# Icelk/fractal-renderer

Measured on AMD Instinct MI355X. Metric: pixel_iterations_per_sec, higher is better.
Workload: dtype f64

## Files before the change

### fractal-renderer_amd/_native.py

```python
import ctypes as C
import os

PKG_DIR = os.path.dirname(os.path.abspath(__file__))
LIB_PATH = os.path.join(PKG_DIR, "libfractal_hip.so")

FR_OK, FR_ERR_INVALID_ARGUMENT, FR_ERR_BUFFER_TOO_SMALL, FR_ERR_NO_DEVICE, FR_ERR_HIP = 0, 1, 2, 3, 4
STATUS_NAMES = {
    1: "FR_ERR_INVALID_ARGUMENT",
    2: "FR_ERR_BUFFER_TOO_SMALL",
    3: "FR_ERR_NO_DEVICE",
    4: "FR_ERR_HIP",
    5: "FR_ERR_UNSUPPORTED_ALGO",
}


class FractalHipError(RuntimeError):
    def __init__(self, code, message):
        super().__init__("%s: %s" % (STATUS_NAMES.get(code, "fr_status %d" % code), message))
        self.code = code


class Imaginary(C.Structure):

    _fields_ = [("re", C.c_double), ("im", C.c_double)]
# ... 241 lines not shown
    "fr_wide_to_double": (C.c_int, [C.c_void_p, C.c_uint32, C.POINTER(C.c_double), C.POINTER(C.c_double)]),
    "fr_wide_from_decimal": (C.c_int, [C.c_char_p, C.c_void_p, C.c_uint32]),
    "fr_render_rows_pt_wide": (
        C.c_int, [C.POINTER(fr_config), _WIDE, C.c_uint32, C.c_uint32, C.c_int, C.c_void_p, C.c_size_t]),
    "fr_render_rows_pt_wide_device": (
        C.c_int, [C.POINTER(fr_config), _WIDE, C.c_uint32, C.c_uint32, C.c_int, C.c_void_p, C.c_size_t, C.c_void_p]),
    "fr_escape_rows_pt_wide": (C.c_int, [C.POINTER(fr_config), _WIDE, C.c_uint32, C.c_uint32, C.c_void_p, C.c_void_p]),
    "fr_escape_rows_pt_wide_state_device": (
        C.c_int,
        [C.POINTER(fr_config), _WIDE, C.c_uint32, C.c_uint32, C.c_void_p, C.c_void_p, C.c_void_p, C.c_void_p, C.c_void_p],
    ),
    "fr_escape_extend_pt_wide_device": (
        C.c_int,
        [C.POINTER(fr_config), _WIDE, C.c_uint32, C.c_uint32, C.c_uint32, C.c_void_p, C.c_void_p, C.c_void_p, C.c_void_p,
         C.c_void_p],
    ),
    "fr_escape_rows_pt_wide_state": (
        C.c_int, [C.POINTER(fr_config), _WIDE, C.c_uint32, C.c_uint32, C.c_void_p, C.c_void_p, C.c_void_p, C.c_void_p]),
    "fr_escape_extend_pt_wide": (
        C.c_int,
        [C.POINTER(fr_config), _WIDE, C.c_uint32, C.c_uint32, C.c_uint32, C.c_void_p, C.c_void_p, C.c_void_p, C.c_void_p],
    ),
    "fr_debug_reference_orbit_wide": (
        C.c_int, [C.POINTER(fr_config), _WIDE, C.c_int, C.c_void_p, C.c_size_t, C.POINTER(C.c_uint32)]),
    "fr_render_rows_pt_bla": (
        C.c_int,
        [C.POINTER(fr_config), C.POINTER(Imaginary), _WIDE, C.c_int, C.c_uint32, C.c_uint32, C.c_int, C.c_void_p, C.c_size_t]),
    "fr_render_rows_pt_bla_device": (
        C.c_int,
        [C.POINTER(fr_config), C.POINTER(Imaginary), _WIDE, C.c_int, C.c_uint32, C.c_uint32, C.c_int, C.c_void_p, C.c_size_t,
         C.c_void_p],
    ),
    "fr_escape_rows_pt_bla": (
        C.c_int, [C.POINTER(fr_config), C.POINTER(Imaginary), _WIDE, C.c_int, C.c_uint32, C.c_uint32, C.c_void_p, C.c_void_p]),
    "fr_escape_rows_pt_bla_device": (
        C.c_int,
        [C.POINTER(fr_config), C.POINTER(Imaginary), _WIDE, C.c_int, C.c_uint32, C.c_uint32, C.c_void_p, C.c_void_p, C.c_void_p],
    ),
    "fr_debug_bla_table": (
        C.c_int,
        [C.POINTER(fr_config), C.POINTER(Imaginary), _WIDE, C.c_int, C.c_int, C.c_uint32, C.c_void_p, C.c_size_t,
         C.POINTER(C.c_uint32)],
    ),
    "fr_debug_bla_count": (
        C.c_int,
        [C.POINTER(fr_config), C.POINTER(Imaginary), _WIDE, C.c_int, C.c_uint32, C.c_uint32, C.POINTER(C.c_uint64),
         C.POINTER(C.c_uint64)],
    ),
    "fr_debug_bla_cache": (C.c_int, [C.POINTER(C.c_uint32)]),
    "fr_render_rows_pt_scaled": (
        C.c_int, [C.POINTER(fr_config), _WIDE, C.c_int, C.c_uint32, C.c_uint32, C.c_int, C.c_void_p, C.c_size_t]),
    "fr_render_rows_pt_scaled_device": (
        C.c_int, [C.POINTER(fr_config), _WIDE, C.c_int, C.c_uint32, C.c_uint32, C.c_int, C.c_void_p, C.c_size_t, C.c_void_p]),
    "fr_escape_rows_pt_scaled": (C.c_int, [C.POINTER(fr_config), _WIDE, C.c_int, C.c_uint32, C.c_uint32, C.c_void_p, C.c_void_p]),
    "fr_escape_rows_pt_scaled_device": (
        C.c_int, [C.POINTER(fr_config), _WIDE, C.c_int, C.c_uint32, C.c_uint32, C.c_void_p, C.c_void_p, C.c_void_p]),
    "fr_debug_bla_table_scaled": (
        C.c_int, [C.POINTER(fr_config), _WIDE, C.c_int, C.c_int, C.c_uint32, C.c_void_p, C.c_size_t, C.POINTER(C.c_uint32)]),
    "fr_debug_pt_scaled_count": (
        C.c_int, [C.POINTER(fr_config), _WIDE, C.c_int, C.c_uint32, C.c_uint32, C.POINTER(C.c_uint64), C.POINTER(C.c_uint64)]),
    "fr_colour_rows_device": (
        C.c_int,
        [C.POINTER(fr_config), C.c_void_p, C.c_int, C.c_void_p, C.c_size_t, C.c_int, C.c_void_p, C.c_size_t, C.c_void_p],
    ),
    "fr_count_iterations": (
        C.c_int,
        [C.POINTER(fr_config), C.c_int, C.c_uint32, C.c_uint32, C.c_uint32, C.c_uint32, C.POINTER(C.c_uint64),
         C.POINTER(C.c_uint64)],
    ),
    "fr_set_profiling": (C.c_int, [C.c_int]),
    "fr_last_kernel_ms": (C.c_int, [C.POINTER(C.c_float)]),
    "fr_set_tile": (C.c_int, [C.c_int]),
    "fr_set_loop_mode": (C.c_int, [C.c_int]),
    "fr_debug_loop_plan": (C.c_int, [C.POINTER(fr_config), C.c_int, C.POINTER(C.c_uint32), C.POINTER(C.c_double),
                                     C.POINTER(C.c_uint32)]),
    "fr_debug_set_spec_maxlen": (C.c_int, [C.c_uint32]),
    "fr_debug_spec_maxlen": (C.c_int, [C.POINTER(fr_config), C.c_int, C.POINTER(C.c_uint32)]),
    "fr_set_palette": (C.c_int, [C.c_int]),
    "fr_set_cycle_shortcut": (C.c_int, [C.c_int]),
    "fr_set_refill_policy": (C.c_int, [C.c_int, C.c_int]),
    "fr_debug_math": (C.c_int, [C.c_int, C.c_void_p, C.c_void_p, C.c_size_t]),
    "fr_debug_set_queue_trace": (C.c_int, [C.c_void_p]),
    "fr_debug_set_two_pass_capacity": (C.c_int, [C.c_uint32]),
}

_lib = None


def load():
    global _lib
    if _lib is not None:
        return _lib
    if not os.path.exists(LIB_PATH):
        raise ImportError(
            "%s is missing — build it first (python -c 'import __graft_entry__ as g; g.build()'); "
            "this package has no CPU fallback" % LIB_PATH
        )
    lib = C.CDLL(LIB_PATH)
    for name, (restype, argtypes) in PROTOTYPES.items():
        fn = getattr(lib, name)
        fn.restype = restype
        fn.argtypes = argtypes
    _lib = lib
    return lib


def check(rc):
    if rc != FR_OK:
        msg = load().fr_last_error()
        raise FractalHipError(rc, msg.decode() if msg else "")
```

### fractal-renderer_amd/build.py

```python
import hashlib
import os
import shutil
import subprocess

PKG_DIR = os.path.dirname(os.path.abspath(__file__))
CSRC = os.path.join(PKG_DIR, "csrc")
LIB_PATH = os.path.join(PKG_DIR, "libfractal_hip.so")
ID_PATH = LIB_PATH + ".id"
KERNEL_SOURCES = ["fr_kernels.hip", "fr_bla.hip", "fr_scaled.hip"]
SOURCES = KERNEL_SOURCES + ["fr_dispatch.hip", "fr_api.hip", "fr_host.hip", "fr_multi.hip", "fr_fern.hip",
                            "fr_dd.hip", "fr_pt.hip", "fr_wide.hip", "fr_ss.hip"]
DEPS = SOURCES + ["fr_kernels.h", "fr_launch.h", "fr_ctx.h", "fr_wide.h", "fr_bla.h", "fr_math.h", "fr_colour.h", "fr_log2_table.inc",
                  os.path.join("..", "..", "include", "fractal_hip.h")]
HIPCC_FLAGS = [
    "--offload-arch=gfx950",
    "-O3",
    "-std=c++17",
    "-ffp-contract=off",
    "-fno-fast-math",
    "-fPIC",
    "-shared",
    "-Wall",
    "-Wextra",
    "-pthread",
]
LINK_FLAGS = ["-ldl"]


def find_hipcc():
    for cand in (os.environ.get("HIPCC"), "/opt/rocm/bin/hipcc", shutil.which("hipcc")):
        if cand and os.path.exists(cand):
            return cand
    raise RuntimeError("hipcc not found (set HIPCC or install ROCm under /opt/rocm)")


def source_id():
    h = hashlib.sha256()
    h.update(" ".join(HIPCC_FLAGS + LINK_FLAGS).encode())
    for d in DEPS:
        h.update(d.encode())
        with open(os.path.join(CSRC, d), "rb") as f:
            h.update(f.read())
    return h.hexdigest()[:16]


def built_id():
    try:
        with open(ID_PATH) as f:
            return f.read().strip()
    except OSError:
        return None


def is_stale():
    return not os.path.exists(LIB_PATH) or built_id() != source_id()


def build_extension(force=False, verbose=False):
    if not force and not is_stale():
        return LIB_PATH
    sid = source_id()
    cmd = ([find_hipcc()] + HIPCC_FLAGS + ['-DFR_BUILD_ID="%s"' % sid, "-o", LIB_PATH]
           + [os.path.join(CSRC, s) for s in SOURCES] + LINK_FLAGS)
    if verbose:
        print(" ".join(cmd))
    if os.path.exists(ID_PATH):
        os.remove(ID_PATH)
    subprocess.run(cmd, check=True, cwd=CSRC)
    with open(ID_PATH, "w") as f:
        f.write(sid + "\n")
    return LIB_PATH


if __name__ == "__main__":
    print(build_extension(force=True, verbose=True))
```

### fractal-renderer_amd/csrc/fr_ctx.h

```cpp
#ifndef FR_CTX_H
#define FR_CTX_H

#include <hip/hip_runtime.h>

#include <atomic>
#include <cstddef>
#include <cstdint>
#include <memory>
#include <condition_variable>
#include <mutex>
#include <string>
#include <thread>
#include <vector>

#include "../../include/fractal_hip.h"
#include "fr_kernels.h"
#include "fr_wide.h"

namespace fr {

int fail(int code, const char *what);
int fail(int code, const std::string &what);
int fail_hip(hipError_t e, const char *what);
const std::string &last_error();
// ... 92 lines not shown
    struct CopyPool *copy_pool = nullptr;
    int reserve_stage(size_t bytes);

    std::mutex pt_mu;
    std::shared_ptr<PtOrbit> pt_orbit;
    std::shared_ptr<BlaTable> bla_table;

    int create(int device);
    void destroy();
    int reserve(Scratch &s, size_t bytes);
    int event(size_t k, hipEvent_t *out);
    int acquire_palette(PaletteSlot **out);
    void release_palette(PaletteSlot *slot, hipStream_t stream);
    int acquire_surv(size_t bytes, SurvSlot **out);
    void release_surv(SurvSlot *slot, hipStream_t stream);
};

void fill_params(const fr_config *cfg, const Opts &o, fr_kparams &p);
void plan_loop(const fr_config *cfg, int precision, const Opts &o, fr_kparams &p);
void rows_params(const fr_config *cfg, const Opts &o, uint32_t y0, uint32_t y1, unsigned channels, fr_kparams &p);

int render_device(Ctx &ctx, const fr_config *cfg, fr_kparams &p, int precision, const Opts &o, void *d_out,
                  hipStream_t stream);

int render_block_cyclic(Ctx &ctx, const fr_config *cfg, int precision, const Opts &o, uint32_t block_rows,
                        uint32_t first_block, uint32_t block_stride, uint32_t max_blocks, int dest_is_image,
                        void *d_out, size_t out_len, hipStream_t stream, uint64_t *rows_written);

int check_precision(int precision);
int check_rows(const fr_config *cfg, uint32_t y0, uint32_t y1);
int check_channels(int channels);

int check_dd(const fr_config *cfg, const fr_imaginary *pos_lo);
int check_pt(const fr_config *cfg, const fr_imaginary *pos_lo);
int check_precision_or_deep(const fr_config *cfg, int precision);
int check_precision_lo(const fr_config *cfg, int precision, const fr_imaginary *pos_lo);

struct Centre {
    const fr_imaginary *pos_lo;
    const fr_wide_centre *wide;
    bool scaled = false;
    double lo_re() const { return pos_lo ? pos_lo->re : 0.0; }
    double lo_im() const { return pos_lo ? pos_lo->im : 0.0; }
    int check(const fr_config *cfg, int precision) const;
};

int prof_begin(hipStream_t stream);
int prof_end(hipStream_t stream, const char *kernel_name);

int render_deep_device(Ctx &ctx, int precision, const fr_config *cfg, const Centre &c, const Opts &o, uint32_t y0, uint32_t y1,
                       unsigned bpp, void *d_out, hipStream_t stream);
int render_rows_device(const fr_config *cfg, int precision, const Centre &c, uint32_t y0, uint32_t y1, void *d_out, size_t out_len,
                       void *hip_stream, unsigned bytes_per_pixel, const fr_render_opts *opts);
int escape_rows(const fr_config *cfg, int precision, const Centre &c, uint32_t y0, uint32_t y1, double *z, uint32_t *iters,
                unsigned zw);
int launch_pt(Ctx &ctx, const fr_config *cfg, const Centre &c, const fr_kparams &p, int mode, const fr_kout &out,
              hipStream_t stream, const char **kernel_name);

struct PtOrbitView {
    const double2 *x = nullptr, *k = nullptr;
    uint32_t x_last = 0, k_last = 0;
};
int pt_orbit_view(Ctx &ctx, const fr_config *cfg, const Centre &c, std::shared_ptr<PtOrbit> &keep, PtOrbitView &v);
void pt_host_orbit(const fr_config *cfg, const Centre &c, int which, std::vector<double> &out);

void decide_kernel(Ctx &ctx, const fr_config *cfg, int precision, uint32_t y0, uint32_t y1, Opts &o, hipStream_t stream,
                   bool allow_async);

int primary(Ctx **out);
Ctx *primary_if_created();

struct LifeShared {
    LifeShared();
    ~LifeShared();
};
struct LifeExclusive {
    LifeExclusive();
    ~LifeExclusive();
};


class ChunkPinner {
  public:
    ChunkPinner(uint8_t *out, size_t need, bool portable, const std::vector<size_t> *byte_order = nullptr);
    ~ChunkPinner();
    size_t chunks() const { return bounds_.size() - 1; }
    size_t bound(size_t k) const { return bounds_[k]; }
    size_t chunk_of(size_t byte) const;
    bool pin(size_t k);
    bool next(size_t &a, size_t &b, bool &pinned);
    void release();
    static size_t chunk_end(const uint8_t *out, size_t need, size_t a);
    double t_touch = 0.0, t_reg = 0.0;

  private:
    uint8_t *out_;
    size_t need_, pos_ = 0;
    unsigned flags_;
    std::vector<size_t> bounds_;
    std::unique_ptr<std::atomic<int>[]> state_;
    std::vector<char> pinned_;
    std::thread toucher_;
    std::mutex reg_mu_;
    std::vector<uint8_t *> regs_;
};
void prefault(void *ptr, size_t len);
void destroy_copy_pool(CopyPool *pool);

struct Profiling {
    bool enabled = false;
    bool have = false;
    hipEvent_t e0 = nullptr, e1 = nullptr;
    const char *kernel = "";
    ~Profiling();
};
Profiling &profiling();


template <class Launch>
int host_rgb(uint8_t *out, size_t need, Launch &&launch) {
    LifeShared ls;
    Ctx *ctx;
    int rc = primary(&ctx);
    if (rc != FR_OK) return rc;
    std::lock_guard<std::mutex> lk(ctx->mu);
    rc = ctx->reserve(ctx->rgb, need);
    if (rc == FR_OK) rc = launch(*ctx, ctx->rgb.ptr, ctx->stream);
    if (rc != FR_OK) return rc;
    HIP_TRY(hipMemcpyAsync(out, ctx->rgb.ptr, need, hipMemcpyDeviceToHost, ctx->stream));
    HIP_TRY(hipStreamSynchronize(ctx->stream));
    return FR_OK;
}

template <class Launch>
int host_raw(double *z, size_t zb, uint32_t *iters, size_t ib, double *dz, uint32_t *m, bool upload, Launch &&launch) {
    LifeShared ls;
    Ctx *ctx;
    int rc = primary(&ctx);
    if (rc != FR_OK) return rc;
    std::lock_guard<std::mutex> lk(ctx->mu);
    if (z) rc = ctx->reserve(ctx->z, dz ? 2 * zb : zb);
    if (rc == FR_OK && iters) rc = ctx->reserve(ctx->iters, m ? 2 * ib : ib);
    if (rc != FR_OK) return rc;
    char *const d_z = z ? static_cast<char *>(ctx->z.ptr) : nullptr, *const d_iters = iters ? static_cast<char *>(ctx->iters.ptr) : nullptr;
    const struct {
        void *host, *dev;
        size_t bytes;
    } arrays[4] = {{z, d_z, zb}, {iters, d_iters, ib}, {dz, dz ? d_z + zb : nullptr, zb}, {m, m ? d_iters + ib : nullptr, ib}};
    if (upload)
        for (const auto &a : arrays)
            if (a.host) HIP_TRY(hipMemcpyAsync(a.dev, a.host, a.bytes, hipMemcpyHostToDevice, ctx->stream));
    rc = launch(*ctx, static_cast<double *>(arrays[0].dev), static_cast<uint32_t *>(arrays[1].dev), static_cast<double *>(arrays[2].dev),
                static_cast<uint32_t *>(arrays[3].dev), ctx->stream);
    if (rc != FR_OK) return rc;
    for (const auto &a : arrays)
        if (a.host) HIP_TRY(hipMemcpyAsync(a.host, a.dev, a.bytes, hipMemcpyDeviceToHost, ctx->stream));
    HIP_TRY(hipStreamSynchronize(ctx->stream));
    return FR_OK;
}

void multi_shutdown_locked();

}

int fr_host_render_rows(const fr_config *cfg, int precision, uint32_t y0, uint32_t y1, uint8_t *out, size_t out_len,
                        unsigned bytes_per_pixel, const fr_render_opts *opts);
int fr_host_render_rows_deep(const fr_config *cfg, int precision, const fr::Centre &c, uint32_t y0, uint32_t y1, uint8_t *out,
                             size_t out_len, unsigned bytes_per_pixel, const fr_render_opts *opts);

#endif
```

### fractal-renderer_amd/csrc/fr_host.hip

```cpp
#include <sys/mman.h>
#include <unistd.h>

#include <immintrin.h>

#include <atomic>
#include <chrono>
#include <condition_variable>
#include <cstdio>
#include <cstdlib>
#include <cstring>
#include <thread>
#include <vector>

#include "fr_ctx.h"

#ifndef MADV_HUGEPAGE
#define MADV_HUGEPAGE 14
#endif

namespace fr {

namespace {

constexpr size_t kPage = 4096;
constexpr size_t kHuge = (size_t)2 << 20;
constexpr size_t kChunk = (size_t)64 << 20;
constexpr size_t kPinThreshold = (size_t)16 << 20;
constexpr size_t kStageMax = (size_t)40 << 20;
constexpr size_t kSdmaMin = (size_t)5 << 20;

double now_ms() {
    using namespace std::chrono;
    return duration<double, std::milli>(steady_clock::now().time_since_epoch()).count();
}

bool trace_enabled() {
    static const bool on = getenv("FR_TRACE") != nullptr;
    return on;
}

int touch_threads() {
    static const int n = [] {
        const char *e = getenv("FR_TOUCH_THREADS");
        if (e && atoi(e) > 0) return atoi(e) > 64 ? 64 : atoi(e);
        long cpus = sysconf(_SC_NPROCESSORS_ONLN);
        return (int)(cpus >= 16 ? 8 : cpus >= 4 ? cpus / 2 : 1);
    }();
    return n;
}

bool looks_resident(uint8_t *p, size_t len) {
    uint8_t *a = reinterpret_cast<uint8_t *>(reinterpret_cast<uintptr_t>(p) & ~(kPage - 1));
    const size_t span = (size_t)(p + len - a);
    const size_t pages = (span + kPage - 1) / kPage;
    std::vector<unsigned char> vec(pages);
    if (mincore(a, span, vec.data()) != 0) return true;
    size_t missing = 0;
    for (size_t k = 0; k < pages; k++) missing += !(vec[k] & 1);
    return missing * 16 < pages;
}

void touch_range(uint8_t *p, size_t len) {
    volatile uint8_t *v = p;
    for (size_t k = 0; k < len; k += kPage) v[k] = v[k];
    if (len) v[len - 1] = v[len - 1];
}

}

void prefault(void *ptr, size_t len) {
    uint8_t *p = static_cast<uint8_t *>(ptr);
    uint8_t *ha = reinterpret_cast<uint8_t *>((reinterpret_cast<uintptr_t>(p) + kHuge - 1) & ~(kHuge - 1));
    uint8_t *hb = reinterpret_cast<uint8_t *>(reinterpret_cast<uintptr_t>(p + len) & ~(kHuge - 1));
    if (hb > ha) (void)madvise(ha, (size_t)(hb - ha), MADV_HUGEPAGE);
    const int T = touch_threads();
    if (T <= 1 || len < 8 * kHuge) {
        touch_range(p, len);
        return;
    }
    std::atomic<size_t> next{0};
    const size_t piece = 4 * kHuge;
    auto work = [&] {
        for (;;) {
            const size_t a = next.fetch_add(piece);
            if (a >= len) break;
            touch_range(p + a, a + piece < len ? piece : len - a);
        }
    };
    std::vector<std::thread> th;
    for (int t = 1; t < T; t++) th.emplace_back(work);
    work();
    for (auto &t : th) t.join();
}


size_t ChunkPinner::chunk_end(const uint8_t *out, size_t need, size_t a) {
    const size_t left = need - a;
    size_t b = a + (left <= kChunk + kChunk / 4 ? kChunk / 4 : kChunk);
    if (b >= need) return need;
    b -= (reinterpret_cast<uintptr_t>(out) + b) & (kPage - 1);
    return b > a ? b : need;
}

ChunkPinner::ChunkPinner(uint8_t *out, size_t need, bool portable, const std::vector<size_t> *byte_order)
    : out_(out), need_(need), flags_(portable ? hipHostRegisterPortable : hipHostRegisterDefault) {
    for (size_t a = 0; a < need;) {
        const size_t b = chunk_end(out, need, a);
        bounds_.push_back(a);
        a = b;
    }
    bounds_.push_back(need);
    const size_t n = chunks();
    state_.reset(new std::atomic<int>[n]);
    const bool fresh = !looks_resident(out, need < 4 * kChunk ? need : 4 * kChunk);
    for (size_t k = 0; k < n; k++) state_[k].store(fresh ? 0 : 1);
    pinned_.assign(n, 0);
    if (fresh) {
        std::vector<size_t> order;
        std::vector<char> seen(n, 0);
        if (byte_order)
            for (size_t byte : *byte_order) {
                const size_t k = chunk_of(byte < need ? byte : need - 1);
                if (!seen[k]) seen[k] = 1, order.push_back(k);
            }
        for (size_t k = 0; k < n; k++)
            if (!seen[k]) order.push_back(k);
        toucher_ = std::thread([this, order] {
            for (size_t k : order) {
                prefault(out_ + bounds_[k], bounds_[k + 1] - bounds_[k]);
                state_[k].store(1, std::memory_order_release);
            }
        });
    }
}

size_t ChunkPinner::chunk_of(size_t byte) const {
    size_t lo = 0, hi = chunks();
    while (hi - lo > 1) {
        const size_t mid = (lo + hi) / 2;
        if (bounds_[mid] <= byte) lo = mid;
        else hi = mid;
    }
    return lo;
}

bool ChunkPinner::pin(size_t k) {
    if (pinned_[k]) return pinned_[k] == 1;
    const uintptr_t base = reinterpret_cast<uintptr_t>(out_);
    const size_t a = bounds_[k], b = bounds_[k + 1];
    const double t0 = now_ms();
    while (state_[k].load(std::memory_order_acquire) == 0) std::this_thread::yield();
    const double t1 = now_ms();
    uint8_t *ra = reinterpret_cast<uint8_t *>((base + a) & ~(kPage - 1));
    uint8_t *rb = b < need_ ? out_ + b : reinterpret_cast<uint8_t *>((base + b + kPage - 1) & ~(kPage - 1));
    const hipError_t re = hipHostRegister(ra, (size_t)(rb - ra), flags_);
    bool ok = re == hipSuccess;
    if (!ok) {
        (void)hipGetLastError();
        ok = re == hipErrorHostMemoryAlreadyRegistered;
    }
    const double t2 = now_ms();
    {
        std::lock_guard<std::mutex> lk(reg_mu_);
        if (re == hipSuccess) regs_.push_back(ra);
        t_touch += t1 - t0;
        t_reg += t2 - t1;
    }
    pinned_[k] = ok ? 1 : 2;
    return ok;
}

bool ChunkPinner::next(size_t &a, size_t &b, bool &pinned) {
    if (pos_ >= chunks()) return false;
    a = bounds_[pos_];
    b = bounds_[pos_ + 1];
    pinned = pin(pos_);
    pos_++;
    return true;
}

void ChunkPinner::release() {
    if (toucher_.joinable()) toucher_.join();
    for (uint8_t *r : regs_) (void)hipHostUnregister(r);
    regs_.clear();
}

ChunkPinner::~ChunkPinner() { release(); }


struct CopyPool {
    struct Piece {
        uint8_t *dst;
        const uint8_t *src;
        size_t len;
        int kind;
    };
    std::vector<std::thread> threads;
    std::mutex m;
    std::condition_variable work_cv, done_cv;
    std::vector<Piece> pieces;
    size_t outstanding = 0;
    bool stop = false;

    explicit CopyPool(int helpers) {
        for (int t = 0; t < helpers; t++) threads.emplace_back([this] { loop(); });
    }
    static void run(const Piece &p) {
        if (p.kind == 0) memcpy(p.dst, p.src, p.len);
        else prefault(p.dst, p.len);
    }
    void loop() {
        for (;;) {
            Piece p;
            {
                std::unique_lock<std::mutex> lk(m);
                work_cv.wait(lk, [&] { return stop || !pieces.empty(); });
                if (pieces.empty()) return;
                p = pieces.back();
                pieces.pop_back();
            }
            run(p);
            std::lock_guard<std::mutex> lk(m);
            if (--outstanding == 0) done_cv.notify_all();
        }
    }
    void post(const std::vector<Piece> &ps) {
        if (ps.empty()) return;
        {
            std::lock_guard<std::mutex> lk(m);
            for (const Piece &p : ps) pieces.push_back(p);
            outstanding += ps.size();
        }
        work_cv.notify_all();
    }
    void wait() {
        for (;;) {
            Piece p;
            {
                std::lock_guard<std::mutex> lk(m);
                if (pieces.empty()) break;
                p = pieces.back();
                pieces.pop_back();
            }
            run(p);
            std::lock_guard<std::mutex> lk(m);
            --outstanding;
        }
        std::unique_lock<std::mutex> lk(m);
        done_cv.wait(lk, [&] { return outstanding == 0; });
    }
    ~CopyPool() {
        {
            std::lock_guard<std::mutex> lk(m);
            stop = true;
        }
        work_cv.notify_all();
        for (auto &t : threads) t.join();
    }
};

void destroy_copy_pool(CopyPool *pool) { delete pool; }

namespace {

// ... 114 lines not shown
    CopyPool *pool = helpers > 0 ? ctx.copy_pool : nullptr;

    auto spread = [&](uint8_t *dst, const uint8_t *src, size_t len, int kind) {
        if (!pool || len < ((size_t)1 << 20)) {
            CopyPool::run(CopyPool::Piece{dst, src, len, kind});
            return;
        }
        const size_t parts = (size_t)helpers + 1;
        const size_t piece = ((len + parts - 1) / parts + 4095) & ~(size_t)4095;
        std::vector<CopyPool::Piece> ps;
        for (size_t off = piece; off < len; off += piece)
            ps.push_back(CopyPool::Piece{dst + off, src ? src + off : nullptr, off + piece < len ? piece : len - off, kind});
        pool->post(ps);
        CopyPool::run(CopyPool::Piece{dst, src, piece < len ? piece : len, kind});
        pool->wait();
    };
    if (rc == FR_OK && err == hipSuccess && need >= ((size_t)1 << 20) && !looks_resident(out, need)) spread(out, nullptr, need, 1);
    const double t_touched = now_ms();
    for (uint32_t b = 0; b < nb && rc == FR_OK && err == hipSuccess; b++) {
        const uint32_t ya = y0 + b * band_rows, yb = ya + band_rows < y1 ? ya + band_rows : y1;
        const size_t a = row_bytes * (size_t)(ya - y0), len = row_bytes * (size_t)(yb - ya);
        if (len < kSdmaMin) {
            err = wait_flag(ctx.stage_flags + b, seq0 + b, (b & 1) ? ctx.stream2 : ctx.stream);
        } else {
            hipEvent_t ec;
            rc = ctx.event(b, &ec);
            if (rc != FR_OK) break;
            err = wait_event(ec);
        }
        if (err != hipSuccess) {
            what = "waiting for a band to arrive in the staging buffer";
            break;
        }
        spread(out + a, stage + a, len, 0);
    }
    if (rc != FR_OK || err != hipSuccess) {
        (void)hipStreamSynchronize(ctx.stream);
        (void)hipStreamSynchronize(ctx.stream2);
        (void)hipStreamSynchronize(ctx.copy_stream);
    }
    if (trace) {
        fprintf(stderr, "[fr_host] staged %zu bytes in %u bands: enqueued at %.3f ms, first touch until %.3f, copied out at %.3f", need, nb,
                t_enqueued - t_start, t_touched - t_start, now_ms() - t_start);
        if (t_enqueued - t_start > 1.0) {
            fprintf(stderr, "  [marks:");
            for (double m : marks) fprintf(stderr, " %.3f", m);
            fprintf(stderr, "]");
        }
        fprintf(stderr, "\n");
    }
    if (rc != FR_OK) return rc;
    if (err != hipSuccess) return fail_hip(err, what);
    return FR_OK;
}


int host_render_rows(Ctx &ctx, const fr_config *cfg, int precision, const Opts &o, uint32_t y0, uint32_t y1,
                     uint8_t *out, unsigned bpp) {
    const size_t row_bytes = (size_t)bpp * cfg->width;
    const size_t need = row_bytes * (size_t)(y1 - y0);
    if (need <= kStageMax && staging_enabled() && ctx.reserve_stage(need > ((size_t)40 << 20) ? need : (size_t)40 << 20) == FR_OK)
        return host_render_staged(ctx, cfg, precision, o, y0, y1, out, bpp);
    int rc = ctx.reserve(ctx.rgb, need);
    if (rc != FR_OK) return rc;
    uint8_t *scratch = static_cast<uint8_t *>(ctx.rgb.ptr);
    const bool trace = trace_enabled();
    const double t_start = now_ms();

    const Opts *use_opts = &o;
    auto render_on = [&](hipStream_t st, uint32_t ya, uint32_t yb, uint8_t *dst) -> int {
        fr_kparams p;
        rows_params(cfg, *use_opts, ya, yb, bpp, p);
        return render_device(ctx, cfg, p, precision, *use_opts, dst, st);
    };

    if (need < kPinThreshold) {
        rc = render_on(ctx.stream, y0, y1, scratch);
        if (rc != FR_OK) return rc;
        HIP_TRY(hipMemcpyAsync(out, scratch, need, hipMemcpyDeviceToHost, ctx.stream));
        HIP_TRY(hipStreamSynchronize(ctx.stream));
        return FR_OK;
    }

    Opts ob = o;
    decide_kernel(ctx, cfg, precision, y0, y1, ob, ctx.stream, true);
    const int pending_sample = ob.pending_sample;
    ob.pending_sample = -1;
    use_opts = &ob;
    struct Band {
        uint32_t ya, yb;
        size_t a, b;
    };
    std::vector<Band> bands;
    {
        uint32_t ya = y0;
        size_t a = 0;
        while (ya < y1) {
            const size_t target = ChunkPinner::chunk_end(out, need, a);
            uint64_t rows = (target - a + row_bytes - 1) / row_bytes;
            rows = (rows + 7) / 8 * 8;
            const uint32_t yb = (uint32_t)((uint64_t)ya + rows < y1 ? ya + rows : y1);
            const size_t b = row_bytes * (size_t)(yb - y0);
            bands.push_back(Band{ya, yb, a, b});
            ya = yb;
            a = b;
        }
    }
    std::vector<size_t> order;
    {
        size_t pow2 = 1;
        int bits = 0;
        while (pow2 < bands.size()) pow2 <<= 1, bits++;
        for (size_t i = 0; i < pow2; i++) {
            size_t r = 0;
            for (int k = 0; k < bits; k++) r |= ((i >> k) & 1u) << (bits - 1 - k);
            if (r < bands.size()) order.push_back(r);
        }
    }
    hipError_t err = hipSuccess;
    const char *what = "";
    std::vector<hipEvent_t> tk, tc;
    hipEvent_t t_zero = nullptr;
    if (trace && hipEventCreate(&t_zero) == hipSuccess) (void)hipEventRecord(t_zero, ctx.stream);
    for (size_t i = 0; i < order.size() && rc == FR_OK && err == hipSuccess; i++) {
        const Band &bd = bands[order[i]];
        hipStream_t st = (i & 1) ? ctx.stream2 : ctx.stream;
        rc = render_on(st, bd.ya, bd.yb, scratch + bd.a);
        if (rc != FR_OK) break;
        hipEvent_t e;
        rc = ctx.event(i, &e);
        if (rc != FR_OK) break;
        if ((err = hipEventRecord(e, st)) != hipSuccess) what = "hipEventRecord";
        if (t_zero) {
            hipEvent_t te;
            if (hipEventCreate(&te) == hipSuccess) {
                (void)hipEventRecord(te, st);
                tk.push_back(te);
            }
        }
    }
    ctx.post_sample(pending_sample, (order.size() & 1) ? ctx.stream : ctx.stream2);
    const double t_launched = now_ms();

    std::vector<size_t> byte_order;
    for (size_t k : order) byte_order.push_back(bands[k].a);
    ChunkPinner pinner(out, need, false, &byte_order);
    for (size_t i = 0; i < order.size() && rc == FR_OK && err == hipSuccess; i++) {
        const Band &bd = bands[order[i]];
        hipEvent_t e;
        rc = ctx.event(i, &e);
        if (rc != FR_OK) break;
        bool waited = false;
        for (size_t pos = bd.a; pos < bd.b && err == hipSuccess;) {
            const size_t k = pinner.chunk_of(pos);
            const size_t end = pinner.bound(k + 1) < bd.b ? pinner.bound(k + 1) : bd.b;
            if (pinner.pin(k)) {
                if (!waited) {
                    if ((err = hipStreamWaitEvent(ctx.copy_stream, e, 0)) != hipSuccess) what = "hipStreamWaitEvent";
                    waited = true;
                }
                if (err == hipSuccess &&
                    (err = hipMemcpyAsync(out + pos, scratch + pos, end - pos, hipMemcpyDeviceToHost, ctx.copy_stream)) != hipSuccess)
                    what = "hipMemcpyAsync";
            } else {
                if ((err = hipEventSynchronize(e)) != hipSuccess) what = "hipEventSynchronize";
                else if ((err = hipMemcpy(out + pos, scratch + pos, end - pos, hipMemcpyDeviceToHost)) != hipSuccess) what = "hipMemcpy";
            }
            pos = end;
        }
        if (t_zero) {
            hipEvent_t te;
            if (hipEventCreate(&te) == hipSuccess) {
                (void)hipEventRecord(te, ctx.copy_stream);
                tc.push_back(te);
            }
        }
    }
    const double t_enqueued = now_ms();
    hipError_t e1 = hipStreamSynchronize(ctx.stream);
    const hipError_t e1b = hipStreamSynchronize(ctx.stream2);
    if (e1 == hipSuccess) e1 = e1b;
    hipError_t e2 = hipStreamSynchronize(ctx.copy_stream);
    const double t_synced = now_ms();
    pinner.release();
    if (trace)
        fprintf(stderr,
                "[fr_host] %zu bytes: kernels enqueued at %.2f ms, waited for first touch %.2f, pinning %.2f, copies "
                "enqueued at %.2f, drained at %.2f, unpinned at %.2f\n",
                need, t_launched - t_start, pinner.t_touch, pinner.t_reg, t_enqueued - t_start, t_synced - t_start,
                now_ms() - t_start);
    if (t_zero) {
        fprintf(stderr, "[fr_host]   band kernels done at (ms):");
        for (hipEvent_t e : tk) {
            float ms = 0.0f;
            (void)hipEventElapsedTime(&ms, t_zero, e);
            fprintf(stderr, " %.1f", ms);
            (void)hipEventDestroy(e);
        }
        fprintf(stderr, "\n[fr_host]   chunk copies done at (ms):");
        for (hipEvent_t e : tc) {
            float ms = 0.0f;
            (void)hipEventElapsedTime(&ms, t_zero, e);
            fprintf(stderr, " %.1f", ms);
            (void)hipEventDestroy(e);
        }
        fprintf(stderr, "\n");
        (void)hipEventDestroy(t_zero);
    }
    if (rc != FR_OK) return rc;
    if (err != hipSuccess) return fail_hip(err, what);
    if (e1 != hipSuccess) return fail_hip(e1, "hipStreamSynchronize(stream)");
    if (e2 != hipSuccess) return fail_hip(e2, "hipStreamSynchronize(copy_stream)");
    return FR_OK;
}

}

using namespace fr;

int fr_host_render_rows(const fr_config *cfg, int precision, uint32_t y0, uint32_t y1, uint8_t *out, size_t out_len,
                        unsigned bpp, const fr_render_opts *opts) {
    int rc = check_rows(cfg, y0, y1);
    if (rc != FR_OK) return rc;
    if (precision == FR_PRECISION_DD || precision == FR_PRECISION_PT)
        return fr_host_render_rows_deep(cfg, precision, Centre{}, y0, y1, out, out_len, bpp, opts);
    rc = check_precision(precision);
    Opts o;
    if (rc == FR_OK) rc = resolve_opts(opts, o);
    if (rc != FR_OK) return rc;
    const size_t need = (size_t)bpp * cfg->width * (size_t)(y1 - y0);
    if (need == 0) return FR_OK;
    if (!out) return fail(FR_ERR_INVALID_ARGUMENT, "out is NULL");
    if (out_len < need)
        return fail(FR_ERR_BUFFER_TOO_SMALL, bpp == 4 ? "out_len < 4*width*(y1-y0)" : "out_len < 3*width*(y1-y0)");
    LifeShared ls;
    Ctx *ctx;
    rc = primary(&ctx);
    if (rc != FR_OK) return rc;
    std::lock_guard<std::mutex> lk(ctx->mu);
    return host_render_rows(*ctx, cfg, precision, o, y0, y1, out, bpp);
}

int fr_host_render_rows_deep(const fr_config *cfg, int precision, const Centre &c, uint32_t y0, uint32_t y1, uint8_t *out,
                             size_t out_len, unsigned bpp, const fr_render_opts *opts) {
    int rc = check_rows(cfg, y0, y1);
    if (rc == FR_OK) rc = c.check(cfg, precision);
    Opts o;
    if (rc == FR_OK) rc = resolve_opts(opts, o);
    if (rc != FR_OK) return rc;
    const size_t need = (size_t)bpp * cfg->width * (size_t)(y1 - y0);
    if (need == 0) return FR_OK;
    if (!out) return fail(FR_ERR_INVALID_ARGUMENT, "out is NULL");
    if (out_len < need)
        return fail(FR_ERR_BUFFER_TOO_SMALL, bpp == 4 ? "out_len < 4*width*(y1-y0)" : "out_len < 3*width*(y1-y0)");
    return host_rgb(out, need, [&](Ctx &ctx, void *d_out, hipStream_t stream) {
        return render_deep_device(ctx, precision, cfg, c, o, y0, y1, bpp, d_out, stream);
    });
}
```

### include/fractal_hip.h

```cpp
#ifndef FRACTAL_HIP_H
#define FRACTAL_HIP_H

#include <stddef.h>
#include <stdint.h>

#ifdef __cplusplus
extern "C" {
#endif

#define FR_ABI_VERSION 3

typedef enum fr_status {
    FR_OK = 0,
    FR_ERR_INVALID_ARGUMENT = 1,
    FR_ERR_BUFFER_TOO_SMALL = 2,
    FR_ERR_NO_DEVICE = 3,
    FR_ERR_HIP = 4,
    FR_ERR_UNSUPPORTED_ALGO = 5
} fr_status;

typedef enum fr_algo {
    FR_ALGO_MANDELBROT = 0,
    FR_ALGO_BARNSLEY_FERN = 1,
    FR_ALGO_JULIA = 2
// ... 220 lines not shown
int fr_wide_from_double(double v, uint64_t *w, uint32_t n);
int fr_wide_add_double(uint64_t *w, uint32_t n, double delta);
int fr_wide_to_double(const uint64_t *w, uint32_t n, double *hi, double *lo);
int fr_wide_from_decimal(const char *text, uint64_t *w, uint32_t n);

int fr_render_rows_pt_wide(const fr_config *cfg, const fr_wide_centre *centre, uint32_t y0, uint32_t y1, int channels,
                           uint8_t *out, size_t out_len);
int fr_render_rows_pt_wide_device(const fr_config *cfg, const fr_wide_centre *centre, uint32_t y0, uint32_t y1, int channels,
                                  void *d_out, size_t out_len, void *hip_stream);
int fr_escape_rows_pt_wide(const fr_config *cfg, const fr_wide_centre *centre, uint32_t y0, uint32_t y1, double *z,
                           uint32_t *iters);
int fr_escape_rows_pt_wide_state_device(const fr_config *cfg, const fr_wide_centre *centre, uint32_t y0, uint32_t y1, void *d_z,
                                        void *d_iters, void *d_dz, void *d_m, void *hip_stream);
int fr_escape_extend_pt_wide_device(const fr_config *cfg, const fr_wide_centre *centre, uint32_t y0, uint32_t y1,
                                    uint32_t from_iterations, void *d_z, void *d_iters, void *d_dz, void *d_m, void *hip_stream);
int fr_escape_rows_pt_wide_state(const fr_config *cfg, const fr_wide_centre *centre, uint32_t y0, uint32_t y1, double *z,
                                 uint32_t *iters, double *dz, uint32_t *m);
int fr_escape_extend_pt_wide(const fr_config *cfg, const fr_wide_centre *centre, uint32_t y0, uint32_t y1, uint32_t from_iterations,
                             double *z, uint32_t *iters, double *dz, uint32_t *m);
int fr_debug_reference_orbit_wide(const fr_config *cfg, const fr_wide_centre *centre, int which, double *out, size_t cap,
                                  uint32_t *len);


int fr_render_rows_pt_bla(const fr_config *cfg, const fr_imaginary *pos_lo, const fr_wide_centre *centre, int bits, uint32_t y0,
                          uint32_t y1, int channels, uint8_t *out, size_t out_len);
int fr_render_rows_pt_bla_device(const fr_config *cfg, const fr_imaginary *pos_lo, const fr_wide_centre *centre, int bits,
                                 uint32_t y0, uint32_t y1, int channels, void *d_out, size_t out_len, void *hip_stream);
int fr_escape_rows_pt_bla(const fr_config *cfg, const fr_imaginary *pos_lo, const fr_wide_centre *centre, int bits, uint32_t y0,
                          uint32_t y1, double *z, uint32_t *iters);
int fr_escape_rows_pt_bla_device(const fr_config *cfg, const fr_imaginary *pos_lo, const fr_wide_centre *centre, int bits,
                                 uint32_t y0, uint32_t y1, void *d_z, void *d_iters, void *hip_stream);
int fr_debug_bla_table(const fr_config *cfg, const fr_imaginary *pos_lo, const fr_wide_centre *centre, int bits, int which,
                       uint32_t level, double *out, size_t cap, uint32_t *len);
int fr_debug_bla_count(const fr_config *cfg, const fr_imaginary *pos_lo, const fr_wide_centre *centre, int bits, uint32_t y0,
                       uint32_t y1, uint64_t *passes, uint64_t *steps);
int fr_debug_bla_cache(uint32_t out[4]);


int fr_render_rows_pt_scaled(const fr_config *cfg, const fr_wide_centre *centre, int bits, uint32_t y0, uint32_t y1, int channels,
                             uint8_t *out, size_t out_len);
int fr_render_rows_pt_scaled_device(const fr_config *cfg, const fr_wide_centre *centre, int bits, uint32_t y0, uint32_t y1,
                                    int channels, void *d_out, size_t out_len, void *hip_stream);
int fr_escape_rows_pt_scaled(const fr_config *cfg, const fr_wide_centre *centre, int bits, uint32_t y0, uint32_t y1, double *z,
                             uint32_t *iters);
int fr_escape_rows_pt_scaled_device(const fr_config *cfg, const fr_wide_centre *centre, int bits, uint32_t y0, uint32_t y1,
                                    void *d_z, void *d_iters, void *hip_stream);
int fr_debug_bla_table_scaled(const fr_config *cfg, const fr_wide_centre *centre, int bits, int which, uint32_t level, double *out,
                              size_t cap, uint32_t *len);
int fr_debug_pt_scaled_count(const fr_config *cfg, const fr_wide_centre *centre, int bits, uint32_t y0, uint32_t y1,
                             uint64_t *passes, uint64_t *steps);


int fr_count_iterations(const fr_config *cfg, int precision, uint32_t y0, uint32_t y1, uint32_t sx,
                        uint32_t sy, uint64_t *total, uint64_t *pixels);

int fr_set_profiling(int enabled);
int fr_last_kernel_ms(float *ms);
int fr_last_kernel_name(char *buf, size_t buf_len);

int fr_set_tile(int tile);

int fr_set_dispatch_sampling(int enabled);
int fr_debug_sample_view(const fr_config *cfg, int precision, double out[8]);
int fr_debug_view_choice(const fr_config *cfg, int precision, uint32_t y0, uint32_t y1, int *state, int *choice,
                         uint32_t *strip_tiles);

int fr_set_refill_policy(int minrun, int quit16);

int fr_set_cycle_shortcut(int enabled);

int fr_set_palette(int enabled);

int fr_set_colour_filter(int enabled);

int fr_set_loop_mode(int mode);
int fr_debug_loop_plan(const fr_config *cfg, int precision, uint32_t *loop_mode, double *skip_t, uint32_t *spec_quiet);
int fr_debug_set_spec_maxlen(uint32_t maxlen);
int fr_debug_spec_maxlen(const fr_config *cfg, int precision, uint32_t *maxlen);

int fr_debug_math(int which, const double *in, double *out, size_t n);
int fr_debug_set_queue_trace(void *d_trace);
int fr_debug_set_two_pass_capacity(uint32_t entries_per_list);

#ifdef __cplusplus
}
#endif
#endif
```

Measured before the change: 5472 billion.

## Pin host chunks on a worker thread and interleave copies with band launches

Moves the host-band planning into a shared header and splits each 64 MiB chunk group into smaller bands (16 MiB by default), so copies can start sooner. The ChunkPinner gets a background thread that registers chunks in band order while kernels launch. Each band's device-to-host copy is now enqueued as soon as its chunks are pinned, instead of after all kernels are launched. The intent is to overlap host registration and D2H transfer with GPU compute, at the cost of more launches, an extra thread, and atomic polling.

```diff
diff --git a/fractal-renderer_amd/_native.py b/fractal-renderer_amd/_native.py
--- a/fractal-renderer_amd/_native.py
+++ b/fractal-renderer_amd/_native.py
@@ -347,6 +347,10 @@
     "fr_debug_math": (C.c_int, [C.c_int, C.c_void_p, C.c_void_p, C.c_size_t]),
     "fr_debug_set_queue_trace": (C.c_int, [C.c_void_p]),
     "fr_debug_set_two_pass_capacity": (C.c_int, [C.c_uint32]),
+    "fr_debug_set_host_band_bytes": (C.c_int, [C.c_size_t]),
+    "fr_debug_plan_host_bands": (C.c_int, [C.c_void_p, C.c_size_t, C.c_size_t, C.c_uint32, C.c_uint32, C.POINTER(C.c_uint64),
+                                           C.POINTER(C.c_uint64), C.POINTER(C.c_uint64), C.POINTER(C.c_uint64), C.c_size_t,
+                                           C.POINTER(C.c_size_t)]),
 }
 
 _lib = None
diff --git a/fractal-renderer_amd/build.py b/fractal-renderer_amd/build.py
--- a/fractal-renderer_amd/build.py
+++ b/fractal-renderer_amd/build.py
@@ -10,7 +10,7 @@
 KERNEL_SOURCES = ["fr_kernels.hip", "fr_bla.hip", "fr_scaled.hip"]
 SOURCES = KERNEL_SOURCES + ["fr_dispatch.hip", "fr_api.hip", "fr_host.hip", "fr_multi.hip", "fr_fern.hip",
                             "fr_dd.hip", "fr_pt.hip", "fr_wide.hip", "fr_ss.hip"]
-DEPS = SOURCES + ["fr_kernels.h", "fr_launch.h", "fr_ctx.h", "fr_wide.h", "fr_bla.h", "fr_math.h", "fr_colour.h", "fr_log2_table.inc",
+DEPS = SOURCES + ["fr_kernels.h", "fr_launch.h", "fr_ctx.h", "fr_bands.h", "fr_wide.h", "fr_bla.h", "fr_math.h", "fr_colour.h", "fr_log2_table.inc",
                   os.path.join("..", "..", "include", "fractal_hip.h")]
 HIPCC_FLAGS = [
     "--offload-arch=gfx950",
diff --git a/fractal-renderer_amd/csrc/fr_bands.h b/fractal-renderer_amd/csrc/fr_bands.h
--- /dev/null
+++ b/fractal-renderer_amd/csrc/fr_bands.h
@@ -0,0 +1,109 @@
+#ifndef FR_BANDS_H
+#define FR_BANDS_H
+
+#include <cstddef>
+#include <cstdint>
+#include <vector>
+
+namespace fr {
+namespace bands {
+
+constexpr size_t kPage = 4096;
+constexpr size_t kChunk = (size_t)64 << 20;
+constexpr size_t kDefaultBandBytes = (size_t)16 << 20;
+
+inline size_t chunk_end(uintptr_t out, size_t need, size_t a) {
+    const size_t left = need - a;
+    size_t b = a + (left <= kChunk + kChunk / 4 ? kChunk / 4 : kChunk);
+    if (b >= need) return need;
+    b -= (size_t)((out + b) & (kPage - 1));
+    return b > a ? b : need;
+}
+
+struct Band {
+    uint32_t ya, yb;
+    size_t a, b;
+    uint32_t group;
+};
+struct Piece {
+    size_t a, b;
+    uint32_t band;
+    uint32_t chunk;
+};
+struct Plan {
+    std::vector<size_t> chunk_bounds;
+    std::vector<Band> bands;
+    std::vector<uint32_t> order;
+    std::vector<Piece> pieces;
+};
+
+inline std::vector<uint32_t> bit_reversed(size_t n) {
+    std::vector<uint32_t> order;
+    size_t pow2 = 1;
+    int bits = 0;
+    while (pow2 < n) pow2 <<= 1, bits++;
+    for (size_t i = 0; i < pow2; i++) {
+        size_t r = 0;
+        for (int k = 0; k < bits; k++) r |= ((i >> k) & 1u) << (bits - 1 - k);
+        if (r < n) order.push_back((uint32_t)r);
+    }
+    return order;
+}
+
+inline Plan plan_host_bands(uintptr_t out, size_t need, size_t row_bytes, uint32_t y0, uint32_t y1, size_t band_bytes) {
+    Plan pl;
+    if (need == 0 || row_bytes == 0 || y1 <= y0) return pl;
+    if (band_bytes == 0) band_bytes = kDefaultBandBytes;
+    for (size_t a = 0; a < need; a = chunk_end(out, need, a)) pl.chunk_bounds.push_back(a);
+    pl.chunk_bounds.push_back(need);
+
+    std::vector<uint32_t> first_band;
+    uint32_t ya = y0;
+    size_t a = 0;
+    while (ya < y1) {
+        const size_t target = chunk_end(out, need, a);
+        uint64_t rows = (target - a + row_bytes - 1) / row_bytes;
+        rows = (rows + 7) / 8 * 8;
+        const uint32_t yg = (uint32_t)((uint64_t)ya + rows < y1 ? ya + rows : y1);
+        const uint64_t grows = yg - ya;
+        uint64_t want = (band_bytes + row_bytes - 1) / row_bytes;
+        want = (want + 7) / 8 * 8;
+        const uint64_t n = (grows + want - 1) / want;
+        const uint64_t brows = ((grows + n - 1) / n + 7) / 8 * 8;
+        const uint32_t g = (uint32_t)first_band.size();
+        first_band.push_back((uint32_t)pl.bands.size());
+        while (ya < yg) {
+            const uint32_t yb = (uint32_t)((uint64_t)ya + brows < yg ? ya + brows : yg);
+            const size_t b = row_bytes * (size_t)(yb - y0);
+            pl.bands.push_back(Band{ya, yb, a, b, g});
+            ya = yb;
+            a = b;
+        }
+    }
+    first_band.push_back((uint32_t)pl.bands.size());
+
+    for (uint32_t g : bit_reversed(first_band.size() - 1))
+        for (uint32_t k = first_band[g]; k < first_band[g + 1]; k++) pl.order.push_back(k);
+
+    for (uint32_t k : pl.order) {
+        const Band &bd = pl.bands[k];
+        size_t lo = 0, hi = pl.chunk_bounds.size() - 1;
+        while (hi - lo > 1) {
+            const size_t mid = (lo + hi) / 2;
+            if (pl.chunk_bounds[mid] <= bd.a) lo = mid;
+            else hi = mid;
+        }
+        for (size_t pos = bd.a; pos < bd.b;) {
+            while (pl.chunk_bounds[lo + 1] <= pos) lo++;
+            const size_t end = pl.chunk_bounds[lo + 1] < bd.b ? pl.chunk_bounds[lo + 1] : bd.b;
+            pl.pieces.push_back(Piece{pos, end, k, (uint32_t)lo});
+            pos = end;
+        }
+    }
+    return pl;
+}
+
+}
+}
+
+#endif
diff --git a/fractal-renderer_amd/csrc/fr_ctx.h b/fractal-renderer_amd/csrc/fr_ctx.h
--- a/fractal-renderer_amd/csrc/fr_ctx.h
+++ b/fractal-renderer_amd/csrc/fr_ctx.h
@@ -198,25 +198,35 @@
 
 class ChunkPinner {
   public:
-    ChunkPinner(uint8_t *out, size_t need, bool portable, const std::vector<size_t> *byte_order = nullptr);
+    ChunkPinner(uint8_t *out, size_t need, bool portable, const std::vector<size_t> *byte_order = nullptr, bool worker = false);
     ~ChunkPinner();
     size_t chunks() const { return bounds_.size() - 1; }
     size_t bound(size_t k) const { return bounds_[k]; }
     size_t chunk_of(size_t byte) const;
     bool pin(size_t k);
+    int ready(size_t k) const { return pinned_[k].load(std::memory_order_acquire); }
     bool next(size_t &a, size_t &b, bool &pinned);
     void release();
     static size_t chunk_end(const uint8_t *out, size_t need, size_t a);
-    double t_touch = 0.0, t_reg = 0.0;
+    double t_touch = 0.0, t_reg = 0.0, t_wait = 0.0;
+    struct WorkerMark {
+        size_t chunk;
+        double t_begin, t_end;
+    };
+    std::vector<WorkerMark> worker_marks;
 
   private:
+    int register_chunk(size_t k, bool by_worker);
     uint8_t *out_;
     size_t need_, pos_ = 0;
     unsigned flags_;
     std::vector<size_t> bounds_;
     std::unique_ptr<std::atomic<int>[]> state_;
-    std::vector<char> pinned_;
-    std::thread toucher_;
+    std::unique_ptr<std::atomic<int>[]> pinned_;
+    std::thread toucher_, worker_;
+    bool has_worker_ = false;
+    std::atomic<bool> stop_{false}, worker_done_{false};
+    double t_epoch_ = 0.0;
     std::mutex reg_mu_;
     std::vector<uint8_t *> regs_;
 };
diff --git a/fractal-renderer_amd/csrc/fr_host.hip b/fractal-renderer_amd/csrc/fr_host.hip
--- a/fractal-renderer_amd/csrc/fr_host.hip
+++ b/fractal-renderer_amd/csrc/fr_host.hip
@@ -12,6 +12,7 @@
 #include <thread>
 #include <vector>
 
+#include "fr_bands.h"
 #include "fr_ctx.h"
 
 #ifndef MADV_HUGEPAGE
@@ -25,6 +26,7 @@
 constexpr size_t kPage = 4096;
 constexpr size_t kHuge = (size_t)2 << 20;
 constexpr size_t kChunk = (size_t)64 << 20;
+static_assert(kPage == bands::kPage && kChunk == bands::kChunk, "fr_bands.h plans with the chunks that ChunkPinner pins");
 constexpr size_t kPinThreshold = (size_t)16 << 20;
 constexpr size_t kStageMax = (size_t)40 << 20;
 constexpr size_t kSdmaMin = (size_t)5 << 20;
@@ -38,6 +40,8 @@
     static const bool on = getenv("FR_TRACE") != nullptr;
     return on;
 }
+
+std::atomic<size_t> g_band_bytes{0};
 
 int touch_threads() {
     static const int n = [] {
@@ -102,7 +106,7 @@
     return b > a ? b : need;
 }
 
-ChunkPinner::ChunkPinner(uint8_t *out, size_t need, bool portable, const std::vector<size_t> *byte_order)
+ChunkPinner::ChunkPinner(uint8_t *out, size_t need, bool portable, const std::vector<size_t> *byte_order, bool worker)
     : out_(out), need_(need), flags_(portable ? hipHostRegisterPortable : hipHostRegisterDefault) {
     for (size_t a = 0; a < need;) {
         const size_t b = chunk_end(out, need, a);
@@ -112,25 +116,40 @@
     bounds_.push_back(need);
     const size_t n = chunks();
     state_.reset(new std::atomic<int>[n]);
+    pinned_.reset(new std::atomic<int>[n]);
     const bool fresh = !looks_resident(out, need < 4 * kChunk ? need : 4 * kChunk);
-    for (size_t k = 0; k < n; k++) state_[k].store(fresh ? 0 : 1);
-    pinned_.assign(n, 0);
-    if (fresh) {
-        std::vector<size_t> order;
-        std::vector<char> seen(n, 0);
-        if (byte_order)
-            for (size_t byte : *byte_order) {
-                const size_t k = chunk_of(byte < need ? byte : need - 1);
-                if (!seen[k]) seen[k] = 1, order.push_back(k);
-            }
-        for (size_t k = 0; k < n; k++)
-            if (!seen[k]) order.push_back(k);
+    for (size_t k = 0; k < n; k++) state_[k].store(fresh ? 0 : 1), pinned_[k].store(0);
+    if (!fresh && !worker) return;
+    std::vector<size_t> order;
+    std::vector<char> seen(n, 0);
+    if (byte_order)
+        for (size_t byte : *byte_order) {
+            const size_t k = chunk_of(byte < need ? byte : need - 1);
+            if (!seen[k]) seen[k] = 1, order.push_back(k);
+        }
+    for (size_t k = 0; k < n; k++)
+        if (!seen[k]) order.push_back(k);
+    if (fresh)
         toucher_ = std::thread([this, order] {
             for (size_t k : order) {
                 prefault(out_ + bounds_[k], bounds_[k + 1] - bounds_[k]);
                 state_[k].store(1, std::memory_order_release);
             }
         });
+    if (worker) {
+        int dev = 0;
+        const bool have_dev = hipGetDevice(&dev) == hipSuccess;
+        if (!have_dev) (void)hipGetLastError();
+        has_worker_ = true;
+        t_epoch_ = now_ms();
+        worker_ = std::thread([this, order, dev, have_dev] {
+            if (have_dev && hipSetDevice(dev) != hipSuccess) (void)hipGetLastError();
+            for (size_t k : order) {
+                if (stop_.load(std::memory_order_acquire)) break;
+                (void)register_chunk(k, true);
+            }
+            worker_done_.store(true, std::memory_order_release);
+        });
     }
 }
 
@@ -144,12 +163,14 @@
     return lo;
 }
 
-bool ChunkPinner::pin(size_t k) {
-    if (pinned_[k]) return pinned_[k] == 1;
+int ChunkPinner::register_chunk(size_t k, bool by_worker) {
     const uintptr_t base = reinterpret_cast<uintptr_t>(out_);
     const size_t a = bounds_[k], b = bounds_[k + 1];
     const double t0 = now_ms();
-    while (state_[k].load(std::memory_order_acquire) == 0) std::this_thread::yield();
+    while (state_[k].load(std::memory_order_acquire) == 0) {
+        if (by_worker && stop_.load(std::memory_order_acquire)) return 0;
+        std::this_thread::yield();
+    }
     const double t1 = now_ms();
     uint8_t *ra = reinterpret_cast<uint8_t *>((base + a) & ~(kPage - 1));
     uint8_t *rb = b < need_ ? out_ + b : reinterpret_cast<uint8_t *>((base + b + kPage - 1) & ~(kPage - 1));
@@ -165,9 +186,24 @@
         if (re == hipSuccess) regs_.push_back(ra);
         t_touch += t1 - t0;
         t_reg += t2 - t1;
-    }
-    pinned_[k] = ok ? 1 : 2;
-    return ok;
+        if (by_worker) worker_marks.push_back(WorkerMark{k, t1 - t_epoch_, t2 - t_epoch_});
+    }
+    const int st = ok ? 1 : 2;
+    pinned_[k].store(st, std::memory_order_release);
+    return st;
+}
+
+bool ChunkPinner::pin(size_t k) {
+    int st = pinned_[k].load(std::memory_order_acquire);
+    if (st == 0 && has_worker_) {
+        const double t0 = now_ms();
+        while ((st = pinned_[k].load(std::memory_order_acquire)) == 0 && !worker_done_.load(std::memory_order_acquire))
+            std::this_thread::yield();
+        if (st == 0) st = pinned_[k].load(std::memory_order_acquire);
+        t_wait += now_ms() - t0;
+    }
+    if (st == 0) st = register_chunk(k, false);
+    return st == 1;
 }
 
 bool ChunkPinner::next(size_t &a, size_t &b, bool &pinned) {
@@ -180,6 +216,8 @@
 }
 
 void ChunkPinner::release() {
+    stop_.store(true, std::memory_order_release);
+    if (worker_.joinable()) worker_.join();
     if (toucher_.joinable()) toucher_.join();
     for (uint8_t *r : regs_) (void)hipHostUnregister(r);
     regs_.clear();
@@ -460,48 +498,61 @@
         return FR_OK;
     }
 
+    const bands::Plan plan = bands::plan_host_bands(reinterpret_cast<uintptr_t>(out), need, row_bytes, y0, y1, g_band_bytes.load());
+    std::vector<size_t> byte_order;
+    for (uint32_t k : plan.order) byte_order.push_back(plan.bands[k].a);
+    const double t_pinner = now_ms();
+    ChunkPinner pinner(out, need, false, &byte_order, true);
+
     Opts ob = o;
     decide_kernel(ctx, cfg, precision, y0, y1, ob, ctx.stream, true);
     const int pending_sample = ob.pending_sample;
     ob.pending_sample = -1;
     use_opts = &ob;
-    struct Band {
-        uint32_t ya, yb;
-        size_t a, b;
-    };
-    std::vector<Band> bands;
-    {
-        uint32_t ya = y0;
-        size_t a = 0;
-        while (ya < y1) {
-            const size_t target = ChunkPinner::chunk_end(out, need, a);
-            uint64_t rows = (target - a + row_bytes - 1) / row_bytes;
-            rows = (rows + 7) / 8 * 8;
-            const uint32_t yb = (uint32_t)((uint64_t)ya + rows < y1 ? ya + rows : y1);
-            const size_t b = row_bytes * (size_t)(yb - y0);
-            bands.push_back(Band{ya, yb, a, b});
-            ya = yb;
-            a = b;
-        }
-    }
-    std::vector<size_t> order;
-    {
-        size_t pow2 = 1;
-        int bits = 0;
-        while (pow2 < bands.size()) pow2 <<= 1, bits++;
-        for (size_t i = 0; i < pow2; i++) {
-            size_t r = 0;
-            for (int k = 0; k < bits; k++) r |= ((i >> k) & 1u) << (bits - 1 - k);
-            if (r < bands.size()) order.push_back(r);
-        }
-    }
+    const size_t nbands = plan.order.size();
     hipError_t err = hipSuccess;
     const char *what = "";
     std::vector<hipEvent_t> tk, tc;
     hipEvent_t t_zero = nullptr;
     if (trace && hipEventCreate(&t_zero) == hipSuccess) (void)hipEventRecord(t_zero, ctx.stream);
-    for (size_t i = 0; i < order.size() && rc == FR_OK && err == hipSuccess; i++) {
-        const Band &bd = bands[order[i]];
+
+    size_t pi = 0;
+    auto copy_band = [&](size_t i, bool wait) -> bool {
+        size_t pe = pi;
+        for (; pe < plan.pieces.size() && plan.pieces[pe].band == plan.order[i]; pe++)
+            if (!wait && pinner.ready(plan.pieces[pe].chunk) != 1) return false;
+        hipEvent_t e;
+        rc = ctx.event(i, &e);
+        if (rc != FR_OK) return true;
+        bool waited = false;
+        for (; pi < pe && err == hipSuccess; pi++) {
+            const bands::Piece &pc = plan.pieces[pi];
+            if (pinner.pin(pc.chunk)) {
+                if (!waited) {
+                    if ((err = hipStreamWaitEvent(ctx.copy_stream, e, 0)) != hipSuccess) what = "hipStreamWaitEvent";
+                    waited = true;
+                }
+                if (err == hipSuccess &&
+                    (err = hipMemcpyAsync(out + pc.a, scratch + pc.a, pc.b - pc.a, hipMemcpyDeviceToHost, ctx.copy_stream)) != hipSuccess)
+                    what = "hipMemcpyAsync";
+            } else {
+                if ((err = hipEventSynchronize(e)) != hipSuccess) what = "hipEventSynchronize";
+                else if ((err = hipMemcpy(out + pc.a, scratch + pc.a, pc.b - pc.a, hipMemcpyDeviceToHost)) != hipSuccess) what = "hipMemcpy";
+            }
+        }
+        if (t_zero) {
+            hipEvent_t te;
+            if (hipEventCreate(&te) == hipSuccess) {
+                (void)hipEventRecord(te, ctx.copy_stream);
+                tc.push_back(te);
+            }
+        }
+        return true;
+    };
+
+    size_t ci = 0;
+    for (size_t i = 0; i < nbands && rc == FR_OK && err == hipSuccess; i++) {
+        const bands::Band &bd = plan.bands[plan.order[i]];
         hipStream_t st = (i & 1) ? ctx.stream2 : ctx.stream;
         rc = render_on(st, bd.ya, bd.yb, scratch + bd.a);
         if (rc != FR_OK) break;
@@ -516,44 +567,11 @@
                 tk.push_back(te);
             }
         }
-    }
-    ctx.post_sample(pending_sample, (order.size() & 1) ? ctx.stream : ctx.stream2);
+        while (ci <= i && rc == FR_OK && err == hipSuccess && copy_band(ci, false)) ci++;
+    }
+    ctx.post_sample(pending_sample, (nbands & 1) ? ctx.stream : ctx.stream2);
     const double t_launched = now_ms();
-
-    std::vector<size_t> byte_order;
-    for (size_t k : order) byte_order.push_back(bands[k].a);
-    ChunkPinner pinner(out, need, false, &byte_order);
-    for (size_t i = 0; i < order.size() && rc == FR_OK && err == hipSuccess; i++) {
-        const Band &bd = bands[order[i]];
-        hipEvent_t e;
-        rc = ctx.event(i, &e);
-        if (rc != FR_OK) break;
-        bool waited = false;
-        for (size_t pos = bd.a; pos < bd.b && err == hipSuccess;) {
-            const size_t k = pinner.chunk_of(pos);
-            const size_t end = pinner.bound(k + 1) < bd.b ? pinner.bound(k + 1) : bd.b;
-            if (pinner.pin(k)) {
-                if (!waited) {
-                    if ((err = hipStreamWaitEvent(ctx.copy_stream, e, 0)) != hipSuccess) what = "hipStreamWaitEvent";
-                    waited = true;
-                }
-                if (err == hipSuccess &&
-                    (err = hipMemcpyAsync(out + pos, scratch + pos, end - pos, hipMemcpyDeviceToHost, ctx.copy_stream)) != hipSuccess)
-                    what = "hipMemcpyAsync";
-            } else {
-                if ((err = hipEventSynchronize(e)) != hipSuccess) what = "hipEventSynchronize";
-                else if ((err = hipMemcpy(out + pos, scratch + pos, end - pos, hipMemcpyDeviceToHost)) != hipSuccess) what = "hipMemcpy";
-            }
-            pos = end;
-        }
-        if (t_zero) {
-            hipEvent_t te;
-            if (hipEventCreate(&te) == hipSuccess) {
-                (void)hipEventRecord(te, ctx.copy_stream);
-                tc.push_back(te);
-            }
-        }
-    }
+    for (; ci < nbands && rc == FR_OK && err == hipSuccess; ci++) (void)copy_band(ci, true);
     const double t_enqueued = now_ms();
     hipError_t e1 = hipStreamSynchronize(ctx.stream);
     const hipError_t e1b = hipStreamSynchronize(ctx.stream2);
@@ -561,12 +579,18 @@
     hipError_t e2 = hipStreamSynchronize(ctx.copy_stream);
     const double t_synced = now_ms();
     pinner.release();
-    if (trace)
+    if (trace) {
         fprintf(stderr,
                 "[fr_host] %zu bytes: kernels enqueued at %.2f ms, waited for first touch %.2f, pinning %.2f, copies "
                 "enqueued at %.2f, drained at %.2f, unpinned at %.2f\n",
                 need, t_launched - t_start, pinner.t_touch, pinner.t_reg, t_enqueued - t_start, t_synced - t_start,
                 now_ms() - t_start);
+        fprintf(stderr, "[fr_host]   %zu bands in %zu chunks; the enqueue waited %.2f ms for pins; pin worker, chunk: registering from-to (ms):",
+                nbands, pinner.chunks(), pinner.t_wait);
+        for (const ChunkPinner::WorkerMark &m : pinner.worker_marks)
+            fprintf(stderr, " %zu: %.2f-%.2f", m.chunk, m.t_begin + t_pinner - t_start, m.t_end + t_pinner - t_start);
+        fprintf(stderr, "\n");
+    }
     if (t_zero) {
         fprintf(stderr, "[fr_host]   band kernels done at (ms):");
         for (hipEvent_t e : tk) {
@@ -635,3 +659,39 @@
         return render_deep_device(ctx, precision, cfg, c, o, y0, y1, bpp, d_out, stream);
     });
 }
+
+
+int fr_debug_set_host_band_bytes(size_t band_bytes) {
+    g_band_bytes.store(band_bytes);
+    return FR_OK;
+}
+
+int fr_debug_plan_host_bands(const void *out, size_t need, size_t row_bytes, uint32_t y0, uint32_t y1, uint64_t *chunk_bounds,
+                             uint64_t *bands_out, uint64_t *order, uint64_t *pieces, size_t cap, size_t counts[4]) {
+    if (!counts) return fail(FR_ERR_INVALID_ARGUMENT, "counts is NULL");
+    if (row_bytes == 0 || y1 <= y0 || need / row_bytes != (size_t)(y1 - y0) || need % row_bytes != 0)
+        return fail(FR_ERR_INVALID_ARGUMENT, "need != row_bytes * (y1 - y0), or no rows");
+    const bands::Plan pl = bands::plan_host_bands(reinterpret_cast<uintptr_t>(out), need, row_bytes, y0, y1, g_band_bytes.load());
+    counts[0] = pl.chunk_bounds.size();
+    counts[1] = pl.bands.size();
+    counts[2] = pl.order.size();
+    counts[3] = pl.pieces.size();
+    for (int k = 0; k < 4; k++)
+        if (counts[k] > cap && (chunk_bounds || bands_out || order || pieces))
+            return fail(FR_ERR_BUFFER_TOO_SMALL, "cap is smaller than one of the plan's lists (see counts)");
+    if (chunk_bounds)
+        for (size_t k = 0; k < pl.chunk_bounds.size(); k++) chunk_bounds[k] = pl.chunk_bounds[k];
+    if (bands_out)
+        for (size_t k = 0; k < pl.bands.size(); k++) {
+            bands_out[4 * k] = pl.bands[k].ya, bands_out[4 * k + 1] = pl.bands[k].yb;
+            bands_out[4 * k + 2] = pl.bands[k].a, bands_out[4 * k + 3] = pl.bands[k].b;
+        }
+    if (order)
+        for (size_t k = 0; k < pl.order.size(); k++) order[k] = pl.order[k];
+    if (pieces)
+        for (size_t k = 0; k < pl.pieces.size(); k++) {
+            pieces[4 * k] = pl.pieces[k].a, pieces[4 * k + 1] = pl.pieces[k].b;
+            pieces[4 * k + 2] = pl.pieces[k].band, pieces[4 * k + 3] = pl.pieces[k].chunk;
+        }
+    return FR_OK;
+}
diff --git a/include/fractal_hip.h b/include/fractal_hip.h
--- a/include/fractal_hip.h
+++ b/include/fractal_hip.h
@@ -326,6 +326,10 @@
 int fr_debug_set_queue_trace(void *d_trace);
 int fr_debug_set_two_pass_capacity(uint32_t entries_per_list);
 
+int fr_debug_set_host_band_bytes(size_t band_bytes);
+int fr_debug_plan_host_bands(const void *out, size_t need, size_t row_bytes, uint32_t y0, uint32_t y1, uint64_t *chunk_bounds,
+                             uint64_t *bands, uint64_t *order, uint64_t *pieces, size_t cap, size_t counts[4]);
+
 #ifdef __cplusplus
 }
 #endif
```

Measured after the change: 5477 billion (median of 2 runs). About the same (+0.1%).
